# Sbte/RAILS

Hardware: AMD Instinct MI355X
Metric: RAILS iterations/sec (+ A*V SpMM HBM GB/s in roofline), m=1M rows/GPU, k=128, fp64 (higher is better)
Workload: dtype f64

## Files before the change

include/rails_hip.h:

```cpp
#ifndef RAILS_HIP_H
#define RAILS_HIP_H

#include <stddef.h>
#include <stdint.h>

#ifdef __cplusplus
extern "C" {
#endif

#define RAILS_OK 0
#define RAILS_EINVAL -1
#define RAILS_EHIP -2
#define RAILS_ENOMEM -3
#define RAILS_ELAPACK -4
#define RAILS_ECOMM -5
#define RAILS_ENODEV -6

typedef struct rails_ctx rails_ctx;
typedef struct rails_csr rails_csr;
typedef struct rails_panel rails_panel;

const char *rails_last_error(void);
const char *rails_version(void);

// ... 87 lines not shown
int rails_csr_gram_norm2_host(int64_t n_rows, int64_t n_cols, const int64_t *rowptr, const int32_t *col, const double *val,
                              const int64_t *t_rowptr, const int32_t *t_col, const double *t_val, double *out);

typedef struct rails_sprhs rails_sprhs;
int rails_sprhs_create(rails_ctx *ctx, int64_t m_local, int p, const int64_t *rowptr, const int32_t *col, const double *val, rails_sprhs **out);
void rails_sprhs_destroy(rails_sprhs *S);
int64_t rails_sprhs_rows(const rails_sprhs *S);
int64_t rails_sprhs_cols(const rails_sprhs *S);
int64_t rails_sprhs_nnz(const rails_sprhs *S);
double rails_sprhs_gram_norm2(const rails_sprhs *S);
int rails_sprhs_apply(rails_ctx *ctx, rails_sprhs *S, int trans, const rails_panel *X, int xc0, int nc, rails_panel *Y, int yc0);
int rails_csr_create_sprhs(rails_ctx *ctx, rails_sprhs *S, rails_csr **out);
int64_t rails_csr_cols(const rails_csr *A);
rails_sprhs *rails_csr_sprhs(const rails_csr *A);


int rails_bsr_count_host(int64_t m, int64_t n_cols, int b, const int64_t *rowptr, const int32_t *col, int64_t *nnzb);
int rails_bsr_fill_host(int64_t m, int64_t n_cols, int b, const int64_t *rowptr, const int32_t *col, const double *val, int64_t *browptr,
                        int32_t *bcol, double *bval);
int rails_bsr_transpose_host(int64_t mb, int64_t nb, int b, const int64_t *browptr, const int32_t *bcol, const double *bval,
                             int64_t *t_browptr, int32_t *t_bcol, double *t_bval);
int rails_csr_create_bsr(rails_ctx *ctx, int64_t mb, int64_t nb_ext, int b, const int64_t *browptr, const int32_t *bcol, const double *bval,
                         rails_csr **out);
int rails_csr_block_size(const rails_csr *A);
int rails_csr_bsr_stats(const rails_csr *A, int64_t *info, int cap);

typedef struct rails_sweep_plan rails_sweep_plan;
int rails_sweep_plan_create(int64_t m, int64_t ncols, const int64_t *rowptr, const int32_t *col, const double *val,
                            const int *params, rails_sweep_plan **out);
int rails_sweep_plan_destroy(rails_sweep_plan *plan);
int rails_sweep_plan_info(const rails_sweep_plan *plan, int64_t *iinfo, double *dinfo);
int rails_sweep_plan_array(const rails_sweep_plan *plan, int which, const void **ptr, int64_t *count);


int rails_panel_create(rails_ctx *ctx, int64_t m_local, int capacity, rails_panel **out);
int rails_panel_create_ld(rails_ctx *ctx, int64_t m_local, int capacity, int ld, rails_panel **out);
int rails_panel_destroy(rails_panel *P);
int64_t rails_panel_rows(const rails_panel *P);
int rails_panel_capacity(const rails_panel *P);
int rails_panel_ld(const rails_panel *P);
void *rails_panel_device_ptr(const rails_panel *P);
int rails_panel_reserve(rails_ctx *ctx, rails_panel *P, int capacity);

int rails_panel_upload(rails_ctx *ctx, rails_panel *P, int c0, int nc, const double *host, int64_t ldh);
int rails_panel_download(rails_ctx *ctx, const rails_panel *P, int c0, int nc, double *host, int64_t ldh);

int rails_panel_fill(rails_ctx *ctx, rails_panel *P, int c0, int nc, double value);
int rails_panel_scale(rails_ctx *ctx, rails_panel *P, int c0, int nc, double s);
int rails_panel_copy(rails_ctx *ctx, const rails_panel *X, int xc0, int nc, rails_panel *Y, int yc0);
int rails_panel_axpy(rails_ctx *ctx, double alpha, const rails_panel *X, int xc0, int nc, rails_panel *Y,
                     int yc0);
int rails_panel_random(rails_ctx *ctx, rails_panel *P, int c0, int nc);

int rails_gram(rails_ctx *ctx, const rails_panel *X, int xc0, int a, const rails_panel *Y, int yc0, int b,
               double *C_host, int ldc);

int rails_panel_gemm(rails_ctx *ctx, double alpha, const rails_panel *X, int xc0, int k, const double *C_host,
                     int ldc, int r, double beta, rails_panel *Y, int yc0);

int rails_ctx_enable_library_gemm(rails_ctx *ctx);
int rails_ctx_library_gemm_ready(const rails_ctx *ctx);

int rails_deferred_reserve(rails_ctx *ctx, int nslots, int64_t doubles_per_slot);
int rails_gram_deferred(rails_ctx *ctx, const rails_panel *X, int xc0, int a, const rails_panel *Y, int yc0, int b, int slot);
int rails_panel_gemm_deferred(rails_ctx *ctx, double alpha, const rails_panel *X, int xc0, int k, int slot, int ld, int r, double beta,
                              rails_panel *Y, int yc0);
int rails_chol_inverse_deferred(rails_ctx *ctx, int slot_in, int w, int slot_out);
int rails_update_gram_deferred(rails_ctx *ctx, double alpha, const rails_panel *X, int xc0, int k, const double *C_host, int ldc, int r,
                               rails_panel *Y, int yc0, int r2, int slot);
int rails_update_gram_deferred_out(rails_ctx *ctx, double alpha, const rails_panel *X, int xc0, int k, const double *C_host, int ldc, int r,
                                   const rails_panel *Y, int yc0, rails_panel *Yout, int oc0, int r2, int slot);
int rails_deferred_fetch(rails_ctx *ctx, int slot, int64_t n, double *host_out);

int rails_panel_gemm_wide(rails_ctx *ctx, double alpha, const rails_panel *X, int xc0, int k, const double *C_host, int ldc, int r,
                          double beta, rails_panel *Y, int yc0);

void rails_dense_set_tile_fit(int on);
int rails_dense_tile_fit(void);
int rails_dense_last_tiles(const rails_ctx *ctx, int *update_gram_nbw, int *gram_cols_ti, int *gemm_wide_tr);

void rails_dense_set_update_gram_pipeline(int on);
int rails_dense_update_gram_pipeline(void);
int rails_dense_last_update_gram_form(const rails_ctx *ctx, int *form);

int rails_orthogonalize(rails_ctx *ctx, rails_panel *V, int k_old, int w, int method, int *used);
int rails_orthogonalize_deflated(rails_ctx *ctx, rails_panel *V, int k_old, int w, const rails_panel *N, int nc0, int q, int method, int *used);

int rails_panel_colnorms2(rails_ctx *ctx, const rails_panel *X, int c0, int nc, double *out_host);

int rails_orthogonalize_range(rails_ctx *ctx, rails_panel *V, int k_old, int w, const rails_panel *N, int nc0, int q, double tol, int *kept,
                              int32_t *kept_idx);

int rails_resid_lanczos(rails_ctx *ctx, const rails_panel *AV, int avc0, const rails_panel *MV, int mvc0, int k,
                        const double *T_host, int ldt, const rails_panel *B, int bc0, int p, int L,
                        double *H_host, int ldh, int *steps);

int rails_resid_lanczos_sparse(rails_ctx *ctx, const rails_panel *AV, int avc0, const rails_panel *MV, int mvc0, int k, const double *T_host,
                               int ldt, const rails_sprhs *S, int L, double *H_host, int ldh, int *steps);

int rails_lanczos_start(rails_ctx *ctx, const rails_panel *AV, int avc0, const rails_panel *MV, int mvc0, int k,
                        const rails_panel *B, int bc0, int p, double *sums_host);

int rails_lanczos_vectors(rails_ctx *ctx, const double *S_host, int lds, int w, rails_panel *Out, int oc0);
int rails_lanczos_last_launch(rails_ctx *ctx, int *nch, int *unroll, int *nblocks);
int rails_lanczos_release(rails_ctx *ctx);

int rails_ctx_reserve_staging(rails_ctx *ctx, size_t bytes);
int rails_timer_start(rails_ctx *ctx);
int rails_timer_stop(rails_ctx *ctx, double *ms);


void rails_sb03md(char dico, char job, char fact, char trans, int n, double *A, int lda, double *X, int ldx,
                  double *scale, int *info);
void rails_sb03md_counts(long *smith, long *schur);
void rails_sb03md_adi_counts(long *extended, long *fresh);
void rails_sb03md_set_pause(int calls);
void rails_dsyev(char jobz, char uplo, int n, double *a, int lda, double *w, int *info);
void rails_dsteqr(char compz, int n, double *d, double *e, double *z, int ldz, double *work, int *info);
void rails_dgemm(char transa, char transb, int m, int n, int k, double alpha, const double *A, int lda, const double *B,
                 int ldb, double beta, double *C, int ldc);
void rails_dtrsm(char side, char uplo, char transa, char diag, int m, int n, double alpha, const double *A, int lda, double *B, int ldb);
void rails_dpotrf(char uplo, int n, double *a, int lda, int *info);
void rails_dpstrf(char uplo, int n, double *a, int lda, int *piv, int *rank, double tol, int *info);
void rails_range_basis(int m, int n, double *a, int lda, double tol, double *q, int ldq, int *rank, int *info);
int rails_host_lapack_init(const char *path);
const char *rails_host_lapack_path(void);

#ifdef __cplusplus
}
#endif
#endif
```

rails_amd/_lib.py:

```python
import ctypes as C
import os

_HERE = os.path.dirname(os.path.abspath(__file__))
LIB_PATH = os.path.join(_HERE, "lib", "librails_hip.so")

_dp = C.POINTER(C.c_double)
_ip = C.POINTER(C.c_int)
_i64p = C.POINTER(C.c_int64)
_i32p = C.POINTER(C.c_int32)
_vp = C.c_void_p

ALLREDUCE_FN = C.CFUNCTYPE(C.c_int, C.c_void_p, C.c_void_p, C.c_size_t, C.c_void_p)
HALO_FN = C.CFUNCTYPE(C.c_int, C.c_void_p, C.c_void_p, C.c_void_p, C.c_int, C.c_void_p)
APPLY_FN = C.CFUNCTYPE(C.c_int, C.c_void_p, C.c_int, C.c_void_p, C.c_int, C.c_int, C.c_void_p, C.c_int)

SIGNATURES = {
    "rails_last_error": (C.c_char_p, []),
    "rails_version": (C.c_char_p, []),
    "rails_ctx_create": (C.c_int, [C.c_int, _vp, C.POINTER(_vp)]),
    "rails_ctx_destroy": (C.c_int, [_vp]),
    "rails_ctx_sync": (C.c_int, [_vp]),
    "rails_ctx_stream": (_vp, [_vp]),
    "rails_ctx_num_cu": (C.c_int, [_vp]),
    "rails_ctx_set_meter": (C.c_int, [_vp, C.c_int]),
# ... 18 lines not shown
    "rails_csr_set_halo_counts": (C.c_int, [_vp, C.c_int, _i64p, _i64p]),
    "rails_csr_create": (C.c_int, [_vp, C.c_int64, C.c_int64, _i64p, _i32p, _dp, C.POINTER(_vp)]),
    "rails_csr_create_rect": (C.c_int, [_vp, C.c_int64, C.c_int64, _i64p, _i32p, _dp, C.POINTER(_vp)]),
    "rails_csr_create_callback": (C.c_int, [_vp, C.c_int64, APPLY_FN, _vp, C.POINTER(_vp)]),
    "rails_csr_destroy": (C.c_int, [_vp]),
    "rails_csr_rows": (C.c_int64, [_vp]),
    "rails_csr_nnz": (C.c_int64, [_vp]),
    "rails_csr_set_halo": (C.c_int, [_vp, C.c_int64, _i64p, C.c_int64, HALO_FN, _vp]),
    "rails_spmm": (C.c_int, [_vp, _vp, C.c_int, _vp, C.c_int, C.c_int, _vp, C.c_int]),
    "rails_csr_set_variant": (C.c_int, [_vp, C.c_int]),
    "rails_csr_sweep_stats": (C.c_int, [_vp, C.c_int, _dp]),
    "rails_csr_tile_stats": (C.c_int, [_vp, _dp]),
    "rails_csr_prepare": (C.c_int, [_vp, _vp, C.c_int, C.c_int, C.POINTER(C.c_int)]),
    "rails_csr_last_kernel": (C.c_char_p, [_vp]),
    "rails_sweep_plan_create": (C.c_int, [C.c_int64, C.c_int64, _i64p, _i32p, _dp, _ip, C.POINTER(_vp)]),
    "rails_sweep_plan_destroy": (C.c_int, [_vp]),
    "rails_sweep_plan_info": (C.c_int, [_vp, _i64p, _dp]),
    "rails_sweep_plan_array": (C.c_int, [_vp, C.c_int, C.POINTER(_vp), _i64p]),
    "rails_panel_create": (C.c_int, [_vp, C.c_int64, C.c_int, C.POINTER(_vp)]),
    "rails_panel_create_ld": (C.c_int, [_vp, C.c_int64, C.c_int, C.c_int, C.POINTER(_vp)]),
    "rails_panel_destroy": (C.c_int, [_vp]),
    "rails_panel_rows": (C.c_int64, [_vp]),
    "rails_panel_capacity": (C.c_int, [_vp]),
    "rails_panel_ld": (C.c_int, [_vp]),
    "rails_panel_device_ptr": (_vp, [_vp]),
    "rails_panel_reserve": (C.c_int, [_vp, _vp, C.c_int]),
    "rails_panel_upload": (C.c_int, [_vp, _vp, C.c_int, C.c_int, _dp, C.c_int64]),
    "rails_panel_download": (C.c_int, [_vp, _vp, C.c_int, C.c_int, _dp, C.c_int64]),
    "rails_panel_fill": (C.c_int, [_vp, _vp, C.c_int, C.c_int, C.c_double]),
    "rails_panel_scale": (C.c_int, [_vp, _vp, C.c_int, C.c_int, C.c_double]),
    "rails_panel_copy": (C.c_int, [_vp, _vp, C.c_int, C.c_int, _vp, C.c_int]),
    "rails_panel_axpy": (C.c_int, [_vp, C.c_double, _vp, C.c_int, C.c_int, _vp, C.c_int]),
    "rails_sptrsv_create": (C.c_int, [_vp, C.c_int64, _i64p, _i32p, _dp, C.c_int, C.c_int, C.POINTER(_vp)]),
    "rails_sptrsv_destroy": (None, [_vp]),
    "rails_sptrsv_levels": (C.c_int64, [_vp]),
    "rails_sptrsv_solve": (C.c_int, [_vp, _vp, _vp, C.c_int, C.c_int]),
    "rails_panel_permute_rows": (C.c_int, [_vp, _vp, C.c_int, C.c_int, _vp, C.c_int, _vp, C.c_int]),
    "rails_index_upload": (C.c_int, [_vp, _i32p, C.c_int64, C.POINTER(_vp)]),
    "rails_index_free": (None, [_vp, _vp]),
    "rails_lu_create": (C.c_int, [_vp, C.c_int64, _i64p, _i32p, _dp, _i64p, _i32p, _dp, _i32p, _i32p, _i32p, C.c_int64, C.POINTER(_vp)]),
    "rails_lu_destroy": (None, [_vp]),
    "rails_lu_solve": (C.c_int, [_vp, _vp, C.c_int, _vp, C.c_int, C.c_int, _vp, C.c_int]),
    "rails_lu_stats": (C.c_int, [_vp, _i64p, C.c_int]),
    "rails_csr_create_lu": (C.c_int, [_vp, _vp, C.POINTER(_vp)]),
    "rails_iter_create": (C.c_int, [_vp, _vp, C.c_int, _dp, C.POINTER(_vp)]),
    "rails_iter_set": (C.c_int, [_vp, C.c_char_p, C.c_double]),
    "rails_iter_solve": (C.c_int, [_vp, _vp, C.c_int, _vp, C.c_int, C.c_int, _vp, C.c_int]),
    "rails_iter_precondition": (C.c_int, [_vp, _vp, _vp, C.c_int, C.c_int, _vp, C.c_int]),
    "rails_iter_amg_setup": (C.c_int, [_vp, _vp]),
    "rails_iter_amg_info": (C.c_int, [_vp, _i64p, _i64p, _dp, C.c_int]),
    "rails_iter_stats": (C.c_int, [_vp, _dp, C.c_int]),
    "rails_iter_columns": (C.c_int, [_vp, _i32p, _dp, _i32p, C.c_int]),
    "rails_csr_create_iter": (C.c_int, [_vp, _vp, C.POINTER(_vp)]),
    "rails_iter_destroy": (None, [_vp]),
    "rails_csr_transpose_host": (C.c_int, [C.c_int64, C.c_int64, _i64p, _i32p, _dp, _i64p, _i32p, _dp]),
    "rails_csr_gram_norm2_host": (C.c_int, [C.c_int64, C.c_int64, _i64p, _i32p, _dp, _i64p, _i32p, _dp, _dp]),
    "rails_bsr_count_host": (C.c_int, [C.c_int64, C.c_int64, C.c_int, _i64p, _i32p, _i64p]),
    "rails_bsr_fill_host": (C.c_int, [C.c_int64, C.c_int64, C.c_int, _i64p, _i32p, _dp, _i64p, _i32p, _dp]),
    "rails_bsr_transpose_host": (C.c_int, [C.c_int64, C.c_int64, C.c_int, _i64p, _i32p, _dp, _i64p, _i32p, _dp]),
    "rails_csr_create_bsr": (C.c_int, [_vp, C.c_int64, C.c_int64, C.c_int, _i64p, _i32p, _dp, C.POINTER(_vp)]),
    "rails_csr_block_size": (C.c_int, [_vp]),
    "rails_csr_bsr_stats": (C.c_int, [_vp, _i64p, C.c_int]),
    "rails_sprhs_create": (C.c_int, [_vp, C.c_int64, C.c_int, _i64p, _i32p, _dp, C.POINTER(_vp)]),
    "rails_sprhs_destroy": (None, [_vp]),
    "rails_sprhs_rows": (C.c_int64, [_vp]),
    "rails_sprhs_cols": (C.c_int64, [_vp]),
    "rails_sprhs_nnz": (C.c_int64, [_vp]),
    "rails_sprhs_gram_norm2": (C.c_double, [_vp]),
    "rails_sprhs_apply": (C.c_int, [_vp, _vp, C.c_int, _vp, C.c_int, C.c_int, _vp, C.c_int]),
    "rails_csr_create_sprhs": (C.c_int, [_vp, _vp, C.POINTER(_vp)]),
    "rails_csr_cols": (C.c_int64, [_vp]),
    "rails_csr_sprhs": (_vp, [_vp]),
    "rails_resid_lanczos_sparse": (C.c_int, [_vp, _vp, C.c_int, _vp, C.c_int, C.c_int, _dp, C.c_int, _vp, C.c_int, _dp, C.c_int, _ip]),
    "rails_panel_random": (C.c_int, [_vp, _vp, C.c_int, C.c_int]),
    "rails_gram": (C.c_int, [_vp, _vp, C.c_int, C.c_int, _vp, C.c_int, C.c_int, _dp, C.c_int]),
    "rails_panel_gemm": (C.c_int, [_vp, C.c_double, _vp, C.c_int, C.c_int, _dp, C.c_int, C.c_int, C.c_double, _vp, C.c_int]),
    "rails_panel_gemm_wide": (C.c_int, [_vp, C.c_double, _vp, C.c_int, C.c_int, _dp, C.c_int, C.c_int, C.c_double, _vp, C.c_int]),
    "rails_dense_set_tile_fit": (None, [C.c_int]),
    "rails_dense_tile_fit": (C.c_int, []),
    "rails_dense_last_tiles": (C.c_int, [_vp, _ip, _ip, _ip]),
    "rails_dense_set_update_gram_pipeline": (None, [C.c_int]),
    "rails_dense_update_gram_pipeline": (C.c_int, []),
    "rails_dense_last_update_gram_form": (C.c_int, [_vp, _ip]),
    "rails_orthogonalize": (C.c_int, [_vp, _vp, C.c_int, C.c_int, C.c_int, _ip]),
    "rails_orthogonalize_deflated": (C.c_int, [_vp, _vp, C.c_int, C.c_int, _vp, C.c_int, C.c_int, C.c_int, _ip]),
    "rails_panel_colnorms2": (C.c_int, [_vp, _vp, C.c_int, C.c_int, _dp]),
    "rails_orthogonalize_range": (C.c_int, [_vp, _vp, C.c_int, C.c_int, _vp, C.c_int, C.c_int, C.c_double, _ip, _i32p]),
    "rails_resid_lanczos": (C.c_int, [_vp, _vp, C.c_int, _vp, C.c_int, C.c_int, _dp, C.c_int, _vp, C.c_int, C.c_int, C.c_int,
                                      _dp, C.c_int, _ip]),
    "rails_lanczos_start": (C.c_int, [_vp, _vp, C.c_int, _vp, C.c_int, C.c_int, _vp, C.c_int, C.c_int, _dp]),
    "rails_lanczos_vectors": (C.c_int, [_vp, _dp, C.c_int, C.c_int, _vp, C.c_int]),
    "rails_lanczos_last_launch": (C.c_int, [_vp, _ip, _ip, _ip]),
    "rails_lanczos_release": (C.c_int, [_vp]),
    "rails_timer_start": (C.c_int, [_vp]),
    "rails_timer_stop": (C.c_int, [_vp, _dp]),
    "rails_sb03md": (None, [C.c_char, C.c_char, C.c_char, C.c_char, C.c_int, _dp, C.c_int, _dp, C.c_int, _dp, _ip]),
    "rails_dsyev": (None, [C.c_char, C.c_char, C.c_int, _dp, C.c_int, _dp, _ip]),
    "rails_dsteqr": (None, [C.c_char, C.c_int, _dp, _dp, _dp, C.c_int, _dp, _ip]),
    "rails_ctx_reserve_staging": (C.c_int, [_vp, C.c_size_t]),
    "rails_sb03md_set_pause": (None, [C.c_int]),
    "rails_sb03md_counts": (None, [C.POINTER(C.c_long), C.POINTER(C.c_long)]),
    "rails_sb03md_adi_counts": (None, [C.POINTER(C.c_long), C.POINTER(C.c_long)]),
    "rails_dtrsm": (None, [C.c_char, C.c_char, C.c_char, C.c_char, C.c_int, C.c_int, C.c_double, _dp, C.c_int, _dp, C.c_int]),
    "rails_dgemm": (None, [C.c_char, C.c_char, C.c_int, C.c_int, C.c_int, C.c_double, _dp, C.c_int, _dp, C.c_int, C.c_double, _dp, C.c_int]),
    "rails_dpotrf": (None, [C.c_char, C.c_int, _dp, C.c_int, _ip]),
    "rails_dpstrf": (None, [C.c_char, C.c_int, _dp, C.c_int, _ip, _ip, C.c_double, _ip]),
    "rails_range_basis": (None, [C.c_int, C.c_int, _dp, C.c_int, C.c_double, _dp, C.c_int, _ip, _ip]),
    "rails_host_lapack_init": (C.c_int, [C.c_char_p]),
    "rails_host_lapack_path": (C.c_char_p, []),
}

_lib = None


class RailsError(RuntimeError):
    pass


def load():
    global _lib
    if _lib is not None:
        return _lib
    if not os.path.exists(LIB_PATH):
        raise RailsError(
            "rails_amd: %s is missing -- build it with `python -c 'import __graft_entry__ as g; g.build()'` "
            "or `make -C rails_amd/csrc`; there is no CPU fallback" % LIB_PATH)
    lib = C.CDLL(LIB_PATH, mode=C.RTLD_GLOBAL)
    for name, (res, args) in SIGNATURES.items():
        fn = getattr(lib, name)
        fn.restype = res
        fn.argtypes = args
    try:
        from ._solver_sigs import bind as _bind_solver
        _bind_solver(lib)
    except ImportError:
        pass
    from ._solution_sigs import bind as _bind_solution

    _bind_solution(lib)
    _lib = lib
    return lib


def check(rc, what=""):
    if rc != 0:
        msg = load().rails_last_error()
        raise RailsError("%s failed (code %d): %s" % (what or "rails call", rc, msg.decode() if msg else ""))
```

rails_amd/csrc/dense_common.h:

```cpp
#pragma once
#include "rails_internal.h"

#include <algorithm>
#include <atomic>

#include "dense_choice.h"

struct DenseSwitch {
    const char *variable;
    int on_by_default;
    std::atomic<int> v{-1};
    bool get()
    {
        if (v.load(std::memory_order_relaxed) < 0) {
            const char *e = getenv(variable);
            int undecided = -1;
            v.compare_exchange_strong(undecided, (e ? atoi(e) : on_by_default) ? 1 : 0);
        }
        return v.load(std::memory_order_relaxed) != 0;
    }
    void set(int on) { v.store(on ? 1 : 0); }
};
extern DenseSwitch g_dense_tile_fit;
extern DenseSwitch g_dense_update_gram_pipeline;

int rails_reduce_partials(rails_ctx *c, const double *partial, int64_t nslab, int64_t n, double *out);

inline int upload_coefficients(rails_ctx *c, const double *C_host, int ldc, int k, int r)
{
    const size_t n = (size_t)k * r;
    RAILS_TRY(rails_small_reserve(c, n * sizeof(double)));
    RAILS_TRY(rails_pinned_begin_write(c, n * sizeof(double)));
    for (int j = 0; j < r; ++j) memcpy(c->pinned + (size_t)j * k, C_host + (size_t)j * ldc, sizeof(double) * k);
    RAILS_HIP_CHECK(hipMemcpyAsync(c->small, c->pinned, n * sizeof(double), hipMemcpyHostToDevice, c->stream));
    return rails_pinned_end_write(c);
}

namespace {

typedef double v4f64 __attribute__((ext_vector_type(4)));
typedef double v2f64 __attribute__((ext_vector_type(2)));

__device__ __forceinline__ v4f64 mfma_f64(double a, double b, v4f64 c)
{
    return __builtin_amdgcn_mfma_f64_16x16x4f64(a, b, c, 0, 0, 0);
}

struct OneSeg {
    const double *X;
    int ld;
    struct Row {
        const double *x;
    };
    __device__ int col(int c) const { return c; }
    __device__ Row row(int64_t r) const { return {X + r * ld}; }
    __device__ static const double *at(Row r, int c) { return r.x + c; }
};
struct TwoSeg {
    const double *X1;
    int ld1, a1;
    const double *X2;
    int ld2;
    struct Col {
        int off;
        bool second;
    };
    struct Row {
        const double *x1, *x2;
    };
    __device__ Col col(int c) const
    {
        const bool second = c >= a1;
        return {second ? c - a1 : c, second};
    }
    __device__ Row row(int64_t r) const { return {X1 + r * ld1, X2 + r * ld2}; }
    __device__ static const double *at(Row r, Col c) { return (c.second ? r.x2 : r.x1) + c.off; }
};

}
```

rails_amd/csrc/dense_gemm.hip:

```cpp
#include "dense_common.h"

#include <dlfcn.h>
#include <mutex>

namespace {

template <int TR, int KC>
__global__ __launch_bounds__(256) void k_panel_gemm(double alpha, const double *X, int ldx, int k,
                                                    const double *__restrict__ C, int r, double beta, double *Yp,
                                                    int ldy, int64_t m, int vec_ok)
{
    const OneSeg Xo{X, ldx};
#define RAILS_PG_VEC4(c) (vec_ok && (c) + 4 <= k)
#include "dense_panel_gemm.inc"
}

template <int TR, int KC>
__global__ __launch_bounds__(256) void k_panel_gemm2(double alpha, const double *X1, int ldx1, int a1, const double *X2, int ldx2, int a,
                                                     const double *__restrict__ C, int r, double beta, double *Yp, int ldy, int64_t m, int vec1,
                                                     int vec2)
{
    const TwoSeg Xo{X1, ldx1, a1, X2, ldx2};
    const int k = a;
#define RAILS_PG_VEC4(c) (((c) + 4 <= a1 && vec1) || ((c) >= a1 && (c) + 4 <= a && vec2))
// ... 21 lines not shown
    const int li = lane & 15, kk = lane >> 4;
    const int64_t r0 = ((int64_t)blockIdx.x * 8 + wave) * 16;
    const int64_t myrow = r0 + li;
    const bool rowok = myrow < m;
    const int nchunks = (k + KC - 1) / KC;
    const uint32_t lds_base = (uint32_t)(uintptr_t)(__attribute__((address_space(3))) unsigned char *)Cs;
    const uint32_t lane16 = (uint32_t)lane * 16u;
    auto stage = [&](int chunk) {
        const char *src = reinterpret_cast<const char *>(Ct) + (size_t)chunk * CHUNK_B;
        const uint32_t dst = lds_base + (uint32_t)((chunk & 1) * CHUNK_B);
        for (int p = wave; p < PIECES; p += 8) {
            uint32_t keep;
            asm volatile("s_mov_b32 %0, m0\n\ts_mov_b32 m0, %3\n\ts_nop 0\n\tglobal_load_lds_dwordx4 %1, %2\n\ts_mov_b32 m0, %0"
                         : "=&s"(keep) : "v"(lane16), "s"(src + (size_t)p * 1024), "s"(dst + (uint32_t)(p * 1024)) : "memory");
        }
    };
    v4f64 acc[TR];
#pragma unroll
    for (int t = 0; t < TR; ++t) acc[t] = (v4f64){0.0, 0.0, 0.0, 0.0};
    const double *xrow = X + (rowok ? myrow : m - 1) * ldx;
    auto fetch = [&](int kcol, double *xs) {
        if (vec_ok && kcol + 4 <= k) {
            v2f64 t0 = *reinterpret_cast<const v2f64 *>(xrow + kcol);
            v2f64 t1 = *reinterpret_cast<const v2f64 *>(xrow + kcol + 2);
            xs[0] = t0.x;
            xs[1] = t0.y;
            xs[2] = t1.x;
            xs[3] = t1.y;
        } else {
#pragma unroll
            for (int s = 0; s < 4; ++s) xs[s] = (kcol + s < k) ? xrow[kcol + s] : 0.0;
        }
    };
    double xa[4], xb[4];
    stage(0);
    fetch(4 * kk, xa);
    fetch(16 + 4 * kk, xb);
    asm volatile("s_waitcnt vmcnt(0)" : : : "memory");
    __builtin_amdgcn_s_barrier();
    for (int ci = 0; ci < nchunks; ++ci) {
        if (ci + 1 < nchunks) stage(ci + 1);
        double xc[4], xd[4];
        fetch((ci + 1) * KC + 4 * kk, xc);
        fetch((ci + 1) * KC + 16 + 4 * kk, xd);
        const double *cb = Cs + (size_t)(ci & 1) * (KC * RL);
#pragma unroll
        for (int s = 0; s < 4; ++s) {
            const double *crow = &cb[(4 * kk + s) * RL + li];
#pragma unroll
            for (int t = 0; t < TR; ++t) acc[t] = mfma_f64(xa[s], crow[16 * t], acc[t]);
        }
        if (!skip_tail || ci * KC + 16 < k) {
#pragma unroll
            for (int s = 0; s < 4; ++s) {
                const double *crow = &cb[(16 + 4 * kk + s) * RL + li];
#pragma unroll
                for (int t = 0; t < TR; ++t) acc[t] = mfma_f64(xb[s], crow[16 * t], acc[t]);
            }
        }
#pragma unroll
        for (int s = 0; s < 4; ++s) {
            xa[s] = xc[s];
            xb[s] = xd[s];
        }
        asm volatile("s_waitcnt vmcnt(0) lgkmcnt(0)" : : : "memory");
        __builtin_amdgcn_s_barrier();
    }
#pragma unroll
    for (int t = 0; t < TR; ++t) {
        const int j = 16 * t + li;
        if (j >= r) continue;
#pragma unroll
        for (int v = 0; v < 4; ++v) {
            const int64_t row = r0 + kk + 4 * v;
            if (row >= m) continue;
            double *dst = Yp + row * ldy + j;
            double val = alpha * acc[t][v];
            if (beta != 0.0) val += beta * (*dst);
            *dst = val;
        }
    }
}

template <int TR>
int launch_pg_wide(rails_ctx *c, double alpha, const double *X, int ldx, int k, const double *C, int r, double beta, double *Y, int ldy, int64_t m, int vec_ok, int skip_tail,
                   double *ct)
{
    constexpr int RL = 16 * TR + 4;
    const int kpad = (k + 31) / 32 * 32;
    RAILS_LAUNCH(k_pack_ct, dim3((unsigned)std::min<int64_t>(512, ((int64_t)kpad * RL + 255) / 256)), dim3(256), 0, c->stream, C, k, r, kpad, RL, ct);
    const size_t lds = (size_t)2 * 32 * RL * sizeof(double);
    RAILS_HIP_CHECK(hipFuncSetAttribute((const void *)k_panel_gemm_wide<TR>, hipFuncAttributeMaxDynamicSharedMemorySize, (int)lds));
    RAILS_LAUNCH((k_panel_gemm_wide<TR>), dim3((unsigned)((m + 127) / 128)), dim3(512), lds, c->stream, alpha, X, ldx, k, ct, r, beta, Y, ldy, m, vec_ok,
                 skip_tail);
    c->last_gemm_wide_tr = TR;
    return RAILS_OK;
}

int scale_only(rails_ctx *c, rails_panel *Y, int yc0, int r, double beta)
{
    if (beta == 0.0) return rails_panel_fill(c, Y, yc0, r, 0.0);
    if (beta == 1.0) return RAILS_OK;
    return rails_panel_scale(c, Y, yc0, r, beta);
}

}

int rails_panel_gemm_dev(rails_ctx *c, double alpha, const double *X, int ldx, int k, const double *C_dev, int r, double beta,
                         double *Y, int ldy, int64_t m)
{
    if (r <= 0 || m <= 0) return RAILS_OK;
    const int vec_ok = dense::rows_vec_ok(X, ldx) ? 1 : 0;
    const dense::PanelGemmChoice p = dense::panel_gemm_choice(r);
    const unsigned grid = (unsigned)((m + 63) / 64);
    switch (p.key()) {
#define RAILS_CASE(TR, KC)                                                                                                                 \
    case dense::inst(TR, KC):                                                                                                              \
        RAILS_LAUNCH((k_panel_gemm<TR, KC>), dim3(grid), dim3(256), 0, c->stream, alpha, X, ldx, k, C_dev, r, beta, Y, ldy, m, vec_ok);    \
        break;
        RAILS_DENSE_PANEL_GEMM_TABLE(RAILS_CASE)
#undef RAILS_CASE
    default: RAILS_REQUIRE(false, "rails_panel_gemm: no k_panel_gemm<%d, %d>", p.tr, p.kc);
    }
    RAILS_HIP_CHECK(hipGetLastError());
    return RAILS_OK;
}

int rails_panel_gemm2_dev(rails_ctx *c, double alpha, const double *X1, int ldx1, int a1, const double *X2, int ldx2, int a2, const double *C_dev,
                          int r, double *Y, int ldy, int64_t m)
{
    if (r <= 0 || m <= 0) return RAILS_OK;
    const int a = a1 + a2;
    const int vec1 = dense::rows_vec_ok(X1, ldx1) ? 1 : 0;
    const int vec2 = (dense::rows_vec_ok(X2, ldx2) && (a1 % 2) == 0) ? 1 : 0;
    const dense::PanelGemmChoice p = dense::panel_gemm2_choice(r);
    const unsigned grid = (unsigned)((m + 63) / 64);
    switch (p.key()) {
#define RAILS_CASE(TR, KC)                                                                                                                 \
    case dense::inst(TR, KC):                                                                                                              \
        RAILS_LAUNCH((k_panel_gemm2<TR, KC>), dim3(grid), dim3(256), 0, c->stream, alpha, X1, ldx1, a1, X2, ldx2, a, C_dev, r, 1.0, Y, ldy, m, vec1, vec2); \
        break;
        RAILS_DENSE_PANEL_GEMM2_TABLE(RAILS_CASE)
#undef RAILS_CASE
    default: RAILS_REQUIRE(false, "rails_panel_gemm2: no k_panel_gemm2<%d, %d>", p.tr, p.kc);
    }
    RAILS_HIP_CHECK(hipGetLastError());
    return RAILS_OK;
}

namespace {
struct RocblasApi {
    void *handle = nullptr;
    int (*create)(void **) = nullptr;
    int (*destroy)(void *) = nullptr;
    int (*set_stream)(void *, hipStream_t) = nullptr;
    int (*dgemm)(void *, int, int, int, int, int, const double *, const double *, int, const double *, int, const double *, double *, int) = nullptr;
    bool tried = false, ok = false;
};
RocblasApi g_rocblas;
std::mutex g_rocblas_mutex;

bool load_rocblas()
{
    std::lock_guard<std::mutex> lock(g_rocblas_mutex);
    if (g_rocblas.tried) return g_rocblas.ok;
    g_rocblas.tried = true;
    const char *e = getenv("RAILS_WIDE_GEMM");
    if (!e || strcmp(e, "rocblas")) return false;
    const char *names[] = {getenv("RAILS_ROCBLAS_LIB"), "librocblas.so", "/opt/rocm/lib/librocblas.so", "librocblas.so.5", "librocblas.so.4"};
    for (const char *n : names) {
        if (!n || !*n) continue;
        if ((g_rocblas.handle = dlopen(n, RTLD_NOW | RTLD_LOCAL))) break;
    }
    if (!g_rocblas.handle) return false;
    g_rocblas.create = (int (*)(void **))dlsym(g_rocblas.handle, "rocblas_create_handle");
    g_rocblas.destroy = (int (*)(void *))dlsym(g_rocblas.handle, "rocblas_destroy_handle");
    g_rocblas.set_stream = (int (*)(void *, hipStream_t))dlsym(g_rocblas.handle, "rocblas_set_stream");
    g_rocblas.dgemm = (decltype(g_rocblas.dgemm))dlsym(g_rocblas.handle, "rocblas_dgemm");
    g_rocblas.ok = g_rocblas.create && g_rocblas.destroy && g_rocblas.set_stream && g_rocblas.dgemm;
    return g_rocblas.ok;
}
constexpr int ROCBLAS_OP_N = 111, ROCBLAS_OP_T = 112;
}

namespace {
struct LibraryGemm {
    std::atomic<int> state{0};
    int device = -1;
    void *handle = nullptr;
    std::mutex use;
};
LibraryGemm g_libgemm;
}

extern "C" int rails_ctx_enable_library_gemm(rails_ctx *c)
{
    RAILS_REQUIRE(c, "rails_ctx_enable_library_gemm: null context");
    std::lock_guard<std::mutex> lock(g_libgemm.use);
    if (g_libgemm.state.load() != 0) return RAILS_OK;
    g_libgemm.device = c->device;
    void *h = nullptr;
    if (!load_rocblas() || hipSetDevice(c->device) != hipSuccess || g_rocblas.create(&h) != 0 || !h) {
        g_libgemm.state = 3;
        return RAILS_OK;
    }
    g_libgemm.handle = h;
    g_libgemm.state = 2;
    return RAILS_OK;
}

extern "C" int rails_ctx_library_gemm_ready(const rails_ctx *c) { return c && g_libgemm.state.load() == 2 && g_libgemm.device == c->device ? 1 : 0; }

extern "C" int rails_panel_gemm_wide(rails_ctx *c, double alpha, const rails_panel *X, int xc0, int k, const double *C_host, int ldc, int r,
                                     double beta, rails_panel *Y, int yc0)
{
    if (c) hipSetDevice(c->device);
    rails_slow_guard slow__(c, "rails_panel_gemm_wide", k, r);
    RAILS_REQUIRE(c && X && Y, "rails_panel_gemm_wide: null argument");
    RAILS_REQUIRE(k >= 0 && r >= 0 && xc0 >= 0 && yc0 >= 0 && xc0 + k <= X->cap && yc0 + r <= Y->cap,
                  "rails_panel_gemm_wide: windows [%d,%d) / [%d,%d) outside capacities %d / %d", xc0, xc0 + k, yc0, yc0 + r, X->cap, Y->cap);
    RAILS_REQUIRE(X->m == Y->m, "rails_panel_gemm_wide: row mismatch %lld vs %lld", (long long)X->m, (long long)Y->m);
    RAILS_REQUIRE(k == 0 || r == 0 || (C_host && ldc >= k), "rails_panel_gemm_wide: bad coefficient matrix (ldc %d < %d)", ldc, k);
    if (X->d == Y->d) RAILS_REQUIRE((xc0 + k <= yc0) || (yc0 + r <= xc0), "rails_panel_gemm_wide: overlapping windows of one panel");
    if (r == 0 || X->m == 0) return RAILS_OK;
    if (k == 0) return scale_only(c, Y, yc0, r, beta);
    RAILS_TRY(upload_coefficients(c, C_host, ldc, k, r));
    if (k >= 64 && r >= 64 && X->m < 0x7fffffffLL && rails_ctx_library_gemm_ready(c)) {
        const int m32 = (int)X->m;
        std::lock_guard<std::mutex> lock(g_libgemm.use);
        int rc = g_rocblas.set_stream(g_libgemm.handle, c->stream);
        if (rc == 0) rc = g_rocblas.dgemm(g_libgemm.handle, ROCBLAS_OP_T, ROCBLAS_OP_N, r, m32, k, &alpha, c->small, k, X->d + xc0, X->ld, &beta, Y->d + yc0, Y->ld);
        if (rc == 0) return RAILS_OK;
        rails_set_error("rails_panel_gemm_wide: rocblas_dgemm failed with status %d", rc);
        return RAILS_EHIP;
    }
    dense::DenseSwitches sw;
    static const int wide_env = spmm_env("RAILS_PANEL_GEMM_WIDE", 1);
    sw.panel_gemm_wide = wide_env;
    sw.tile_fit = g_dense_tile_fit.get();
    const dense::GemmWidePlan plan = dense::gemm_wide_plan(k, r, sw);
    if (!plan.own_kernel) {
        for (int j0 = 0; j0 < r; j0 += 128) {
            const int nc = std::min(128, r - j0);
            RAILS_TRY(rails_panel_gemm_dev(c, alpha, X->d + xc0, X->ld, k, c->small + (size_t)j0 * k, nc, beta, Y->d + yc0 + j0, Y->ld, X->m));
        }
        return RAILS_OK;
    }
    const int vec_ok = dense::rows_vec_ok(X->d + xc0, X->ld) ? 1 : 0;
    RAILS_TRY(rails_ws_reserve(c, (size_t)plan.nslices * plan.ct_doubles * sizeof(double)));
    for (int j = 0; j < plan.count(); ++j) {
        const dense::GemmWideSlice s = plan.slice(j);
        const double *Cj = c->small + (size_t)s.j0 * k;
        double *Yj = Y->d + yc0 + s.j0, *ct = c->ws + (size_t)j * plan.ct_doubles;
        switch (s.tr) {
#define RAILS_CASE(TR)                                                                                                                     \
    case TR:                                                                                                                               \
        RAILS_TRY((launch_pg_wide<TR>(c, alpha, X->d + xc0, X->ld, k, Cj, s.nc, beta, Yj, Y->ld, X->m, vec_ok, plan.tile_fit ? 1 : 0, ct))); \
        break;
            RAILS_DENSE_GEMM_WIDE_TABLE(RAILS_CASE)
#undef RAILS_CASE
        default: RAILS_REQUIRE(false, "rails_panel_gemm_wide: no k_panel_gemm_wide<%d>", s.tr);
        }
    }
    RAILS_HIP_CHECK(hipGetLastError());
    return RAILS_OK;
}

extern "C" int rails_panel_gemm(rails_ctx *c, double alpha, const rails_panel *X, int xc0, int k, const double *C_host, int ldc,
                                int r, double beta, rails_panel *Y, int yc0)
{
    if (c) hipSetDevice(c->device);
    rails_slow_guard slow__(c, "rails_panel_gemm", k, r);
    RAILS_REQUIRE(c && X && Y, "rails_panel_gemm: null argument");
    RAILS_REQUIRE(k >= 0 && r >= 0 && xc0 >= 0 && yc0 >= 0 && xc0 + k <= X->cap && yc0 + r <= Y->cap,
                  "rails_panel_gemm: windows [%d,%d) / [%d,%d) outside capacities %d / %d", xc0, xc0 + k, yc0, yc0 + r, X->cap, Y->cap);
    RAILS_REQUIRE(X->m == Y->m, "rails_panel_gemm: row mismatch %lld vs %lld", (long long)X->m, (long long)Y->m);
    RAILS_REQUIRE(r <= 256, "rails_panel_gemm: r = %d > 256 output columns per call", r);
    RAILS_REQUIRE(k == 0 || r == 0 || (C_host && ldc >= k), "rails_panel_gemm: bad coefficient matrix (ldc %d < %d)", ldc, k);
    if (X->d == Y->d) {
        bool same = (xc0 == yc0);
        bool disjoint = (xc0 + k <= yc0) || (yc0 + r <= xc0);
        RAILS_REQUIRE(same || disjoint, "rails_panel_gemm: partially overlapping windows of one panel");
    }
    if (r == 0 || X->m == 0) return RAILS_OK;
    if (k == 0) return scale_only(c, Y, yc0, r, beta);
    RAILS_TRY(upload_coefficients(c, C_host, ldc, k, r));
    return rails_panel_gemm_dev(c, alpha, X->d + xc0, X->ld, k, c->small, r, beta, Y->d + yc0, Y->ld, X->m);
}
```

rails_amd/csrc/rails_internal.h:

```cpp
#ifndef RAILS_INTERNAL_H
#define RAILS_INTERNAL_H

#include <hip/hip_runtime.h>

#include <cstdarg>
#include <cstdint>
#include <cstdio>
#include <cstring>
#include <ctime>
#include <string>
#include <vector>

#include "rails_hip.h"

void rails_set_error(const char *fmt, ...);

#define RAILS_HIP_CHECK(expr)                                                                      \
    do {                                                                                           \
        hipError_t e__ = (expr);                                                                   \
        if (e__ != hipSuccess) {                                                                   \
            rails_set_error("%s:%d: %s failed: %s", __FILE__, __LINE__, #expr, hipGetErrorString(e__)); \
            return RAILS_EHIP;                                                                     \
        }                                                                                          \
    } while (0)

#define RAILS_REQUIRE(cond, ...)                                                                   \
    do {                                                                                           \
        if (!(cond)) {                                                                             \
            rails_set_error(__VA_ARGS__);                                                          \
            return RAILS_EINVAL;                                                                   \
        }                                                                                          \
    } while (0)

#define RAILS_TRY(expr)                                                                            \
    do {                                                                                           \
        int rc__ = (expr);                                                                         \
        if (rc__ != RAILS_OK) return rc__;                                                         \
    } while (0)

static inline int rails_pad_ld(int capacity) { return ((capacity < 1 ? 1 : capacity) + 15) / 16 * 16; }

struct rails_ctx {
    int device = 0;
    hipStream_t stream = nullptr;
    bool own_stream = false;
    hipStream_t stream2 = nullptr;
    hipEvent_t ev_fork = nullptr, ev_join = nullptr;
    int num_cu = 256;
    uint64_t seed = 1;
    uint64_t next_stream = 0;
    int rank = 0, nranks = 1;
    int64_t row0 = 0, m_global = -1;
    rails_allreduce_fn allreduce = nullptr;
    void *allreduce_user = nullptr;
    void *rccl = nullptr;
    bool own_rccl = false;
    int rccl_nranks = 0, rccl_rank = 0;
    double *ws = nullptr;
    size_t ws_bytes = 0;
    std::vector<std::pair<size_t, double *>> free_panels;
    size_t free_panel_bytes = 0;
    double *small = nullptr;
    size_t small_bytes = 0;
    double *pinned = nullptr;
    size_t pinned_bytes = 0;
    hipEvent_t ev0 = nullptr, ev1 = nullptr;
    hipEvent_t ev_h2d = nullptr;
    bool h2d_pending = false;
    double *defer_dev = nullptr, *defer_pin = nullptr;
    size_t defer_slot = 0;
    int defer_nslots = 0;
    bool meter = false;
    std::vector<hipEvent_t> meter_events;
    int meter_open = 0;
    long meter_missed = 0;
    double gpu_busy_ms = 0.0;
    void *lz = nullptr;
    long n_orth_block = 0, n_orth_columnwise = 0, n_spmm_tiled = 0, n_spmm_planes = 0, n_spmm_overlapped = 0, n_spmm_sweep = 0, n_spmm_rowgather = 0, n_spmm_callback = 0, n_dev_alloc = 0, n_allreduce = 0, n_lanczos = 0, n_lanczos_start = 0, n_orth_repair = 0, n_update_gram_fused = 0, n_rowquad = 0;
    long n_orth_range = 0, n_orth_range_passes = 0, n_orth_range_syncs = 0;
    int last_update_gram_nbw = 0, last_gram_cols_ti = 0, last_gemm_wide_tr = 0;
    int last_update_gram_form = 0;
    int last_rowquad_nslices = 0, last_rowquad_tr[2] = {0, 0};
};

constexpr int RAILS_METER_PAIRS = 512;
inline bool rails_meter_before(rails_ctx *c)
{
    if (!c->meter) return false;
    if (c->meter_open >= RAILS_METER_PAIRS) {
        c->meter_missed++;
        return false;
    }
    hipEventRecord(c->meter_events[2 * c->meter_open], c->stream);
    return true;
}
inline void rails_meter_after(rails_ctx *c) { hipEventRecord(c->meter_events[2 * c->meter_open++ + 1], c->stream); }
inline hipError_t rails_stream_sync(rails_ctx *c)
{
    const hipError_t e = hipStreamSynchronize(c->stream);
    for (int i = 0; i < c->meter_open; ++i) {
        float ms = 0.0f;
        if (e == hipSuccess && hipEventElapsedTime(&ms, c->meter_events[2 * i], c->meter_events[2 * i + 1]) == hipSuccess) c->gpu_busy_ms += ms;
    }
    c->meter_open = 0;
    return e;
}
#define RAILS_LAUNCH(...)                                                                                                                  \
    do {                                                                                                                                   \
        const bool rails_metered = rails_meter_before(c);                                                                                  \
        hipLaunchKernelGGL(__VA_ARGS__);                                                                                                   \
        if (rails_metered) rails_meter_after(c);                                                                                           \
    } while (0)

struct rails_panel {
    rails_ctx *ctx = nullptr;
    double *d = nullptr;
    int64_t m = 0;
    int cap = 0;
    int ld = 0;
};

struct rails_planes_plan;
struct rails_sweep_cache;
struct rails_tile_cache;
struct rails_bsr;

struct rails_csr {
    rails_ctx *ctx = nullptr;
    rails_sweep_cache *sweep = nullptr;
    rails_planes_plan *planes = nullptr;
    rails_tile_cache *tiled = nullptr;
    int64_t m = 0, ncols_ext = 0, nnz = 0;
    bool rect = false;
    int64_t *rowptr = nullptr;
    int32_t *col = nullptr;
    double *val = nullptr;
    int max_row_nnz = 0;
    int64_t window_rows = 0;
    rails_csr *AT = nullptr;
    std::vector<int64_t> h_rowptr;
    std::vector<int32_t> h_col;
    std::vector<double> h_val;
    int64_t n_send = 0, n_ghost = 0;
    int64_t int_lo = 0, int_hi = 0;
    int64_t window_rows_int = 0;
    int64_t *send_rows = nullptr;
    double *send_buf = nullptr;
    double *ext = nullptr;
    size_t send_cap = 0, ext_cap = 0;
    rails_halo_fn halo = nullptr;
    void *halo_user = nullptr;
    std::vector<int64_t> send_counts, recv_counts;
    int variant = 0;
    int is_grid = -1;
    const char *last_kernel = "";
    enum Kind { STORED, CALLBACK, LU, SPRHS, ITER, BSR } kind = STORED;
    void *delegate = nullptr;
    rails_apply_fn apply_fn = nullptr;
    rails_lu *lu() const { return kind == LU ? static_cast<rails_lu *>(delegate) : nullptr; }
    rails_sprhs *sprhs() const { return kind == SPRHS ? static_cast<rails_sprhs *>(delegate) : nullptr; }
    rails_iter *iter() const { return kind == ITER ? static_cast<rails_iter *>(delegate) : nullptr; }
    rails_bsr *bsr() const { return kind == BSR ? static_cast<rails_bsr *>(delegate) : nullptr; }
};
// ... 99 lines not shown
```

Measured before the change: 243.7.

## Add software-pipelined wide panel GEMM with LDS-DMA staging of coefficient chunks

Adds a new wide panel GEMM kernel that double-buffers the packed coefficient matrix in LDS using global_load_lds direct-to-LDS loads. It also prefetches the next chunk of X row values into registers while the MFMA work on the current chunk runs. The point is to overlap global loads with FP64 MFMA compute and take the staging copy off the VGPR path. The new kernel is on by default behind an environment switch, and it relies on inline asm that manipulates m0 and on explicit waitcnt/barrier placement, which could be fragile.

```diff
diff --git a/include/rails_hip.h b/include/rails_hip.h
--- a/include/rails_hip.h
+++ b/include/rails_hip.h
@@ -193,6 +193,10 @@
 void rails_dense_set_update_gram_pipeline(int on);
 int rails_dense_update_gram_pipeline(void);
 int rails_dense_last_update_gram_form(const rails_ctx *ctx, int *form);
+
+void rails_dense_set_gemm_wide_pipeline(int on);
+int rails_dense_gemm_wide_pipeline(void);
+int rails_dense_last_gemm_wide_form(const rails_ctx *ctx, int *form);
 
 int rails_orthogonalize(rails_ctx *ctx, rails_panel *V, int k_old, int w, int method, int *used);
 int rails_orthogonalize_deflated(rails_ctx *ctx, rails_panel *V, int k_old, int w, const rails_panel *N, int nc0, int q, int method, int *used);
diff --git a/rails_amd/_lib.py b/rails_amd/_lib.py
--- a/rails_amd/_lib.py
+++ b/rails_amd/_lib.py
@@ -124,6 +124,9 @@
     "rails_dense_set_update_gram_pipeline": (None, [C.c_int]),
     "rails_dense_update_gram_pipeline": (C.c_int, []),
     "rails_dense_last_update_gram_form": (C.c_int, [_vp, _ip]),
+    "rails_dense_set_gemm_wide_pipeline": (None, [C.c_int]),
+    "rails_dense_gemm_wide_pipeline": (C.c_int, []),
+    "rails_dense_last_gemm_wide_form": (C.c_int, [_vp, _ip]),
     "rails_orthogonalize": (C.c_int, [_vp, _vp, C.c_int, C.c_int, C.c_int, _ip]),
     "rails_orthogonalize_deflated": (C.c_int, [_vp, _vp, C.c_int, C.c_int, _vp, C.c_int, C.c_int, C.c_int, _ip]),
     "rails_panel_colnorms2": (C.c_int, [_vp, _vp, C.c_int, C.c_int, _dp]),
diff --git a/rails_amd/csrc/dense_common.h b/rails_amd/csrc/dense_common.h
--- a/rails_amd/csrc/dense_common.h
+++ b/rails_amd/csrc/dense_common.h
@@ -23,6 +23,7 @@
 };
 extern DenseSwitch g_dense_tile_fit;
 extern DenseSwitch g_dense_update_gram_pipeline;
+extern DenseSwitch g_dense_gemm_wide_pipeline;
 
 int rails_reduce_partials(rails_ctx *c, const double *partial, int64_t nslab, int64_t n, double *out);
 
diff --git a/rails_amd/csrc/dense_gemm.hip b/rails_amd/csrc/dense_gemm.hip
--- a/rails_amd/csrc/dense_gemm.hip
+++ b/rails_amd/csrc/dense_gemm.hip
@@ -127,18 +127,139 @@
     }
 }
 
+template <int TR, bool VEC>
+__global__ __launch_bounds__(512) void k_panel_gemm_wide_p(double alpha, const double *__restrict__ X, int ldx, int k, const double *__restrict__ Ct ,
+                                                           int r, double beta, double *__restrict__ Yp, int ldy, int64_t m, int skip_tail)
+{
+    constexpr int KC = 32, RL = 16 * TR + 4, CHUNK_B = KC * RL * 8, PIECES = CHUNK_B / 1024;
+    static_assert(CHUNK_B % 1024 == 0, "whole LDS-DMA pieces per chunk");
+    extern __shared__ double Cs[];
+    const int lane = threadIdx.x & 63;
+    const int wave = __builtin_amdgcn_readfirstlane((int)(threadIdx.x >> 6));
+    const int li = lane & 15, kk = lane >> 4;
+    const int64_t r0 = ((int64_t)blockIdx.x * 8 + wave) * 16;
+    const int64_t myrow = r0 + li;
+    const bool rowok = myrow < m;
+    const int nchunks = (k + KC - 1) / KC;
+    const int steady = std::max(k / KC - 1, 0);
+    const uint32_t lds_base = (uint32_t)(uintptr_t)(__attribute__((address_space(3))) unsigned char *)Cs;
+    const uint32_t lane16 = (uint32_t)lane * 16u;
+    auto stage = [&](int chunk) {
+        const char *src = reinterpret_cast<const char *>(Ct) + (size_t)chunk * CHUNK_B;
+        const uint32_t dst = lds_base + (uint32_t)((chunk & 1) * CHUNK_B);
+        for (int p = wave; p < PIECES; p += 8) {
+            uint32_t keep;
+            asm volatile("s_mov_b32 %0, m0\n\ts_mov_b32 m0, %3\n\ts_nop 0\n\tglobal_load_lds_dwordx4 %1, %2\n\ts_mov_b32 m0, %0"
+                         : "=&s"(keep) : "v"(lane16), "s"(src + (size_t)p * 1024), "s"(dst + (uint32_t)(p * 1024)) : "memory");
+        }
+    };
+    v4f64 acc[TR];
+#pragma unroll
+    for (int t = 0; t < TR; ++t) acc[t] = (v4f64){0.0, 0.0, 0.0, 0.0};
+    const double *xrow = X + (rowok ? myrow : m - 1) * ldx;
+    auto fetch_inside = [&](int kcol, double *xs) {
+        if constexpr (VEC) {
+            v2f64 t0 = *reinterpret_cast<const v2f64 *>(xrow + kcol);
+            v2f64 t1 = *reinterpret_cast<const v2f64 *>(xrow + kcol + 2);
+            xs[0] = t0.x;
+            xs[1] = t0.y;
+            xs[2] = t1.x;
+            xs[3] = t1.y;
+        } else {
+#pragma unroll
+            for (int s = 0; s < 4; ++s) xs[s] = xrow[kcol + s];
+        }
+    };
+    auto fetch_edge = [&](int kcol, double *xs) {
+#pragma unroll
+        for (int s = 0; s < 4; ++s) {
+            const double v = xrow[std::min(kcol + s, k - 1)];
+            xs[s] = (kcol + s < k) ? v : 0.0;
+        }
+    };
+    double xa[4], xb[4];
+    auto step = [&](int ci, double *xc, double *xd, bool whole) {
+        const double *cb = Cs + (size_t)(ci & 1) * (KC * RL);
+#pragma unroll
+        for (int s = 0; s < 4; ++s) {
+            const double *crow = &cb[(4 * kk + s) * RL + li];
+#pragma unroll
+            for (int t = 0; t < TR; ++t) acc[t] = mfma_f64(xa[s], crow[16 * t], acc[t]);
+        }
+        if (whole || !skip_tail || ci * KC + 16 < k) {
+#pragma unroll
+            for (int s = 0; s < 4; ++s) {
+                const double *crow = &cb[(16 + 4 * kk + s) * RL + li];
+#pragma unroll
+                for (int t = 0; t < TR; ++t) acc[t] = mfma_f64(xb[s], crow[16 * t], acc[t]);
+            }
+        }
+#pragma unroll
+        for (int s = 0; s < 4; ++s) {
+            xa[s] = xc[s];
+            xb[s] = xd[s];
+        }
+        asm volatile("s_waitcnt vmcnt(0) lgkmcnt(0)" : : : "memory");
+        __builtin_amdgcn_s_barrier();
+    };
+    stage(0);
+    fetch_edge(4 * kk, xa);
+    fetch_edge(16 + 4 * kk, xb);
+    asm volatile("s_waitcnt vmcnt(0)" : : : "memory");
+    __builtin_amdgcn_s_barrier();
+    int ci = 0;
+    for (; ci < steady; ++ci) {
+        stage(ci + 1);
+        double xc[4], xd[4];
+        fetch_inside((ci + 1) * KC + 4 * kk, xc);
+        fetch_inside((ci + 1) * KC + 16 + 4 * kk, xd);
+        __builtin_amdgcn_sched_barrier(0);
+        step(ci, xc, xd, true);
+    }
+    for (; ci < nchunks; ++ci) {
+        if (ci + 1 < nchunks) stage(ci + 1);
+        double xc[4], xd[4];
+        fetch_edge((ci + 1) * KC + 4 * kk, xc);
+        fetch_edge((ci + 1) * KC + 16 + 4 * kk, xd);
+        step(ci, xc, xd, false);
+    }
+#pragma unroll
+    for (int t = 0; t < TR; ++t) {
+        const int j = 16 * t + li;
+        if (j >= r) continue;
+#pragma unroll
+        for (int v = 0; v < 4; ++v) {
+            const int64_t row = r0 + kk + 4 * v;
+            if (row >= m) continue;
+            double *dst = Yp + row * ldy + j;
+            double val = alpha * acc[t][v];
+            if (beta != 0.0) val += beta * (*dst);
+            *dst = val;
+        }
+    }
+}
+
 template <int TR>
 int launch_pg_wide(rails_ctx *c, double alpha, const double *X, int ldx, int k, const double *C, int r, double beta, double *Y, int ldy, int64_t m, int vec_ok, int skip_tail,
-                   double *ct)
+                   bool pipeline, double *ct)
 {
     constexpr int RL = 16 * TR + 4;
     const int kpad = (k + 31) / 32 * 32;
     RAILS_LAUNCH(k_pack_ct, dim3((unsigned)std::min<int64_t>(512, ((int64_t)kpad * RL + 255) / 256)), dim3(256), 0, c->stream, C, k, r, kpad, RL, ct);
     const size_t lds = (size_t)2 * 32 * RL * sizeof(double);
-    RAILS_HIP_CHECK(hipFuncSetAttribute((const void *)k_panel_gemm_wide<TR>, hipFuncAttributeMaxDynamicSharedMemorySize, (int)lds));
-    RAILS_LAUNCH((k_panel_gemm_wide<TR>), dim3((unsigned)((m + 127) / 128)), dim3(512), lds, c->stream, alpha, X, ldx, k, ct, r, beta, Y, ldy, m, vec_ok,
-                 skip_tail);
+    const dim3 grid((unsigned)((m + 127) / 128));
+    if (!pipeline) {
+        RAILS_HIP_CHECK(hipFuncSetAttribute((const void *)k_panel_gemm_wide<TR>, hipFuncAttributeMaxDynamicSharedMemorySize, (int)lds));
+        RAILS_LAUNCH((k_panel_gemm_wide<TR>), grid, dim3(512), lds, c->stream, alpha, X, ldx, k, ct, r, beta, Y, ldy, m, vec_ok, skip_tail);
+    } else if (vec_ok) {
+        RAILS_HIP_CHECK(hipFuncSetAttribute((const void *)k_panel_gemm_wide_p<TR, true>, hipFuncAttributeMaxDynamicSharedMemorySize, (int)lds));
+        RAILS_LAUNCH((k_panel_gemm_wide_p<TR, true>), grid, dim3(512), lds, c->stream, alpha, X, ldx, k, ct, r, beta, Y, ldy, m, skip_tail);
+    } else {
+        RAILS_HIP_CHECK(hipFuncSetAttribute((const void *)k_panel_gemm_wide_p<TR, false>, hipFuncAttributeMaxDynamicSharedMemorySize, (int)lds));
+        RAILS_LAUNCH((k_panel_gemm_wide_p<TR, false>), grid, dim3(512), lds, c->stream, alpha, X, ldx, k, ct, r, beta, Y, ldy, m, skip_tail);
+    }
     c->last_gemm_wide_tr = TR;
+    c->last_gemm_wide_form = pipeline ? 2 : 1;
     return RAILS_OK;
 }
 
@@ -292,6 +413,7 @@
         return RAILS_OK;
     }
     const int vec_ok = dense::rows_vec_ok(X->d + xc0, X->ld) ? 1 : 0;
+    const bool pipeline = g_dense_gemm_wide_pipeline.get();
     RAILS_TRY(rails_ws_reserve(c, (size_t)plan.nslices * plan.ct_doubles * sizeof(double)));
     for (int j = 0; j < plan.count(); ++j) {
         const dense::GemmWideSlice s = plan.slice(j);
@@ -300,7 +422,7 @@
         switch (s.tr) {
 #define RAILS_CASE(TR)                                                                                                                     \
     case TR:                                                                                                                               \
-        RAILS_TRY((launch_pg_wide<TR>(c, alpha, X->d + xc0, X->ld, k, Cj, s.nc, beta, Yj, Y->ld, X->m, vec_ok, plan.tile_fit ? 1 : 0, ct))); \
+        RAILS_TRY((launch_pg_wide<TR>(c, alpha, X->d + xc0, X->ld, k, Cj, s.nc, beta, Yj, Y->ld, X->m, vec_ok, plan.tile_fit ? 1 : 0, pipeline, ct))); \
         break;
             RAILS_DENSE_GEMM_WIDE_TABLE(RAILS_CASE)
 #undef RAILS_CASE
@@ -308,6 +430,19 @@
         }
     }
     RAILS_HIP_CHECK(hipGetLastError());
+    return RAILS_OK;
+}
+
+DenseSwitch g_dense_gemm_wide_pipeline{"RAILS_GEMM_WIDE_PIPELINE", 1};
+
+extern "C" void rails_dense_set_gemm_wide_pipeline(int on) { g_dense_gemm_wide_pipeline.set(on); }
+
+extern "C" int rails_dense_gemm_wide_pipeline(void) { return g_dense_gemm_wide_pipeline.get() ? 1 : 0; }
+
+extern "C" int rails_dense_last_gemm_wide_form(const rails_ctx *c, int *form)
+{
+    RAILS_REQUIRE(c && form, "rails_dense_last_gemm_wide_form: null argument");
+    *form = c->last_gemm_wide_form;
     return RAILS_OK;
 }
 
diff --git a/rails_amd/csrc/rails_internal.h b/rails_amd/csrc/rails_internal.h
--- a/rails_amd/csrc/rails_internal.h
+++ b/rails_amd/csrc/rails_internal.h
@@ -79,6 +79,7 @@
     long n_orth_block = 0, n_orth_columnwise = 0, n_spmm_tiled = 0, n_spmm_planes = 0, n_spmm_overlapped = 0, n_spmm_sweep = 0, n_spmm_rowgather = 0, n_spmm_callback = 0, n_dev_alloc = 0, n_allreduce = 0, n_lanczos = 0, n_lanczos_start = 0, n_orth_repair = 0, n_update_gram_fused = 0, n_rowquad = 0;
     long n_orth_range = 0, n_orth_range_passes = 0, n_orth_range_syncs = 0;
     int last_update_gram_nbw = 0, last_gram_cols_ti = 0, last_gemm_wide_tr = 0;
+    int last_gemm_wide_form = 0;
     int last_update_gram_form = 0;
     int last_rowquad_nslices = 0, last_rowquad_tr[2] = {0, 0};
 };
```

New measurement: 242.9. About the same (-0.3%).
